# Rongjiehuang/FastDiff

Hardware: AMD Instinct MI355X
Metric: real-time factor (audio-sec/wall-sec), N=4 reverse steps, 80x864 mel (higher is better)
Workload: dtype f32 results; 2-piece fp16 operands (22 bit) on fp16 MFMA, fp32 accumulate; GEMM as Winograd F(2,3); exact-fp32 twin; 1 GPU; BASELINE configs[1]: LJSpeech shape, batch=8 x 80x864 mel per GPU, N=4, HIP kernels + hipGraph sampler; batch_per_gpu=8, frames=864, reverse_steps=4, graph=True, weights=random init seed 1234 (no checkpoint offline), world_size=1, gpus_visible=1, oversubscribed=False

## Files before the change

### fastdiff_amd/csrc/fd_api.cpp

```cpp
#include <math.h>
#include <stddef.h>
#include <stdio.h>
#include <stdlib.h>
#include <string.h>

#include <algorithm>

#include "fd_kernels.h"
#include "fd_host.h"

std::string g_create_error;

static inline int gx_rows_host(int T) { return std::max(fdk_fast::gx_rows(T), fdk_fast::gw_pairs(T) * (fdk_fast::GW_ROWB / fdk_fast::GX_ROWB)); }

bool fd_prof_stamps(const fdk::Launch &L, const char *name, hipEvent_t *e0, hipEvent_t *e1)
{
    fd_context *c = L.ctx;
    if (c->profile != 1 || L.capturing) return false;
    hipEvent_t ev[2];
    for (int i = 0; i < 2; ++i) {
        if (!c->event_pool.empty()) { ev[i] = c->event_pool.back(); c->event_pool.pop_back(); }
        else if (hipEventCreate(&ev[i]) != hipSuccess) return false;
    }
    ProfEntry pe;
// ... 300 lines not shown
    }
    for (int i = fuse_up ? 1 : 0; i < fd::LAYERS; ++i) {
        if (m.fast[ST_LVC]) {
            e = fast_lvc_layer(L, io, n, i, cur, skip, other, B, T);
            std::swap(cur, other);
        } else {
            e = naive_lvc_layer(L, n, i, cur, skip, other, B, T);
        }
        if (e != hipSuccess) return e;
    }
    if (m.keep_taps) {
        e = hipMemcpyAsync(ws.xtap[n], cur, sizeof(float) * (size_t)B * fd::C * T * fd::hop(n), hipMemcpyDeviceToDevice, L.stream);
        if (e != hipSuccess) return e;
    }
    *x_out = cur;
    return hipSuccess;
}

static hipError_t run_step(const Launch &L, const StepIO &io, int B, int T)
{
    Workspace &ws = L.ctx->ws;
    hipError_t e;
    const bool hoisted = L.mode->hoist_np > 1;
    if ((e = first_conv(L, io, B, T)) != hipSuccess) return e;
    for (int d = 0; d < fd::NBLK; ++d)
        if ((e = dblock(L, io, d, B, T)) != hipSuccess) return e;
    if (!hoisted) {
        if ((e = kp_front(L, io, B, T)) != hipSuccess) return e;
        if ((e = kp_gemm(L, B, T)) != hipSuccess) return e;
    }
    float *x = ws.a[3];
    for (int n = 0; n < fd::NBLK; ++n) {
        float *xo = nullptr;
        if ((e = lvc_block_run(L, io, n, x, B, T, &xo)) != hipSuccess) return e;
        x = xo;
    }
    if (L.mode->fast[ST_FINAL]) return fast_final(L, io, x, B, T);
    float *eps = io.sampler ? ((x == ws.xA) ? ws.xB : ws.xA) : io.eps_out;
    if ((e = naive_final_eps(L, x, eps, B, T)) != hipSuccess) return e;
    if (io.sampler) return naive_update(L, ws.x, eps, (int64_t)B * T * fd::HOPT);
    return hipSuccess;
}

}

extern "C" {


// ... 103 lines not shown
    if (e != hipSuccess) FD_FAIL(h, FD_ERR_HIP, "fd_forward: kernel launch failed: %s", hipGetErrorString(e));
    h->last_B = B; h->last_T = T;
    return fd_mark_tail(h, (hipStream_t)stream);
}

static int resolve_pending(fd_handle h, unsigned *mask);
int fd_settle(fd_handle h)
{
    if (!h->pending.active) return FD_OK;
    unsigned mask = 0;
    const int rc = resolve_pending(h, &mask);
    return rc < 0 ? rc : FD_OK;
}

static int enqueue_steps(fd_handle h, int B, int T, int count, const StepMode &mode, hipStream_t stream)
{
    Workspace &ws = h->ws;
    constexpr int CHUNK = 8;
    auto piece_mode = [&](int steps) {
        StepMode m = mode;
        if (m.hoist_chunk) m.hoist_np = steps;
        return m;
    };
    const bool defer_advance = mode.fuse_advance && mode.fast[ST_FIRST];
    auto enqueue_piece = [&](const fdk::Launch &L, int steps) -> hipError_t {
        const int np = L.mode->hoist_chunk ? L.mode->hoist_np : 1;
        hipError_t e = hipSuccess;
        if (np > 1) {
            StepIO iop = {ws.x, ws.mel_rep, nullptr, nullptr, np};
            e = fdk::kp_front(L, iop, B * np, T);
            if (e == hipSuccess) e = fdk::kp_gemm(L, B * np, T);
        }
        for (int k = 0; k < steps && e == hipSuccess; ++k) {
            StepIO io = {ws.x, ws.mel, nullptr, nullptr, 1};
            io.hoist_step = L.mode->hoist_np > 1 ? k : 0;
            io.advance = k > 0 && defer_advance;
            e = fdk::run_step(L, io, B, T);
            if (e == hipSuccess && !(k + 1 < steps && defer_advance)) e = fdk::advance_step(L);
        }
        return e;
    };
    if (!(h->use_graph && !h->profile)) {
        const int piece = mode.hoist_chunk ? CHUNK : count;
        for (int first = 0; first < count; first += piece) {
            const int steps = std::min(piece, count - first);
            const StepMode m = piece_mode(steps);
            const hipError_t e = enqueue_piece({h, stream, false, &m}, steps);
// ... 363 lines not shown
    static const char *stage_names[ST_COUNT] = {"embed", "first", "dblock", "kp_front", "kp_gemm", "convt", "lvc", "final"};
    auto parse_mode = [&](bool &dst) -> int {
        if (v == "fast") dst = true;
        else if (v == "naive") dst = false;
        else FD_FAIL(h, FD_ERR_INVALID, "fd_set_option: %s expects fast|naive, got '%s'", key, value);
        return FD_OK;
    };
    if (k == "kernels") {
        bool m = true;
        int rc = parse_mode(m);
        if (rc != FD_OK) return rc;
        for (int i = 0; i < ST_COUNT; ++i) h->mode.fast[i] = m;
        return FD_OK;
    }
    if (k.compare(0, 8, "kernels.") == 0) {
        for (int i = 0; i < ST_COUNT; ++i)
            if (k.substr(8) == stage_names[i]) return parse_mode(h->mode.fast[i]);
        FD_FAIL(h, FD_ERR_INVALID, "fd_set_option: unknown stage '%s'", key);
    }
    static const struct { const char *key, *a, *b; void (*set)(fd_context *, bool); } choices[] = {
        {"gemm", "f16x2", "fp32", [](fd_context *c, bool a) { c->mode.gemm_f16 = a; }},
        {"gemm_form", "winograd", "direct", [](fd_context *c, bool a) { c->mode.gemm_wino = a; }},
        {"gemm_tile", "16", "32", [](fd_context *c, bool a) { c->mode.gemm_tile16 = a; }},
        {"lvc", "f16x2", "fp32", [](fd_context *c, bool a) { c->mode.lvc_f16 = a; }},
        {"conv", "f16x2", "fp32", [](fd_context *c, bool a) { c->mode.conv_f16 = a; }},
        {"lvc_h8", "mfma", "valu", [](fd_context *c, bool a) { c->mode.lvc_h8_mfma = a; }},
        {"fallback", "graph", "host", [](fd_context *c, bool a) { c->host_fallback = !a; }},
        {"lvc_dx", "gather", "copy", [](fd_context *c, bool a) { c->lvc_dx_gather = a; }},
        {"mel", "pwg", "tacotron", [](fd_context *c, bool a) { c->mel_variant = a ? MEL_PWG : MEL_TACOTRON; }},
    };
    for (const auto &ch : choices) {
        if (k != ch.key) continue;
        if (v != ch.a && v != ch.b) FD_FAIL(h, FD_ERR_INVALID, "fd_set_option: %s expects %s|%s, got '%s'", key, ch.a, ch.b, value);
        ch.set(h, v == ch.a);
        return FD_OK;
    }
    const bool on = (v == "1" || v == "true" || v == "on");
    if (k == "fuse_final") { h->mode.fuse_final = on; return FD_OK; }
    if (k == "fuse_up") { h->mode.fuse_up = on; return FD_OK; }
    if (k == "fuse_advance") { h->mode.fuse_advance = on; return FD_OK; }
    if (k == "embed_cache") { h->embed_cache = on; return FD_OK; }
    if (k == "hoist") {
        if (v == "auto") h->hoist_mode = 1;
        else if (v == "on") h->hoist_mode = 2;
        else if (v == "off") h->hoist_mode = 0;
        else FD_FAIL(h, FD_ERR_INVALID, "fd_set_option: hoist expects auto|on|off, got '%s'", value);
// ... 20 lines not shown
```

### fastdiff_amd/csrc/fd_internal.h

```cpp
#pragma once
#include <hip/hip_runtime.h>
#include <hip/hip_ext.h>
#include <stdint.h>
#include <string.h>
#include <map>
#include <string>
#include <vector>

#include "../../include/fastdiff_hip.h"
#include "../../include/fastdiff_hip_ext.h"
#include "../../include/fastdiff_hip_train.h"

namespace fd {
constexpr int C = 32;
constexpr int COND = 80;
constexpr int HID = 64;
constexpr int NBLK = 3;
constexpr int LAYERS = 4;
constexpr int HOPT = 256;
constexpr int E_IN = 128, E_MID = 512, E_OUT = 512;
constexpr int KLAYER = 2 * C * C * 3;
constexpr int KW = KLAYER * LAYERS;
constexpr int KB = 2 * C * LAYERS;
constexpr int KREC = KW + KB;
// ... 58 lines not shown
    int n_steps;
    int ddim;
    int step_idx;
    int l4;
    const unsigned long long *uids;
    int l4_io;
    long long n4_io;
    const long long *offs4;
};

enum Stage { ST_EMBED = 0, ST_FIRST, ST_DBLOCK, ST_KP_FRONT, ST_KP_GEMM, ST_CONVT, ST_LVC, ST_FINAL, ST_COUNT };

struct StepMode {
    bool fast[ST_COUNT] = {true, true, true, true, true, true, true, true};
    bool gemm_f16 = true;
    bool gemm_wino = true;
    bool gemm_tile16 = true;
    bool lvc_f16 = true;
    bool conv_f16 = true;
    bool lvc_h8_mfma = true;
    bool fuse_final = true;
    bool fuse_up = true;
    bool fuse_advance = true;
    bool keep_taps = false;
    unsigned fp32_mask = 0;
    bool inline_fallback = true;
    bool ragged = false;
    int hoist_np = 1;
    bool hoist_chunk = false;

    bool operator==(const StepMode &o) const
    {
        for (int i = 0; i < ST_COUNT; ++i)
            if (fast[i] != o.fast[i]) return false;
        return gemm_f16 == o.gemm_f16 && gemm_wino == o.gemm_wino && gemm_tile16 == o.gemm_tile16 && lvc_f16 == o.lvc_f16 && conv_f16 == o.conv_f16 &&
               lvc_h8_mfma == o.lvc_h8_mfma && fuse_final == o.fuse_final && fuse_up == o.fuse_up && fuse_advance == o.fuse_advance &&
               keep_taps == o.keep_taps && fp32_mask == o.fp32_mask && inline_fallback == o.inline_fallback && ragged == o.ragged &&
               hoist_np == o.hoist_np && hoist_chunk == o.hoist_chunk;
    }
};

struct Workspace {
    int B = 0;
    int64_t frames = 0;
    int64_t rows = 0;
    float *noise = nullptr;
    float *embed_h2 = nullptr;
    float *a[4] = {};
    float *kp_h0 = nullptr, *kp_hA = nullptr, *kp_hB = nullptr;
    float *kpack = nullptr;
    float *h_f16 = nullptr;
    int *lens_dev = nullptr;
    unsigned long long *uid_dev = nullptr;
    long long *off_dev = nullptr;
    float *xsave = nullptr;
    int *range_flag = nullptr;
    float *xA = nullptr, *xB = nullptr;
    float *xtap[fd::NBLK] = {};
    int64_t pframes = 0, prows = 0, plens = 0;
    float *mel_rep = nullptr;
// ... 135 lines not shown
    Scratch step_scratch;
    std::vector<ProfEntry> prof_pending;
    std::vector<hipEvent_t> event_pool;
    std::map<std::string, std::pair<int64_t, double>> prof_acc;
};

enum Pipe { PIPE_F16_THEN_F32, PIPE_F16_ONLY, PIPE_F32_ONLY };
inline Pipe fd_pipe(const StepMode &m, bool f16_possible, int flag_word)
{
    if (!f16_possible || ((m.fp32_mask >> flag_word) & 1u)) return PIPE_F32_ONLY;
    return m.inline_fallback ? PIPE_F16_THEN_F32 : PIPE_F16_ONLY;
}
inline bool front_writes_h_image(const StepMode &m, const DevWeights &w)
{
    return m.fast[ST_KP_FRONT] && fd_pipe(m, m.conv_f16 && w.kpf_f16_ok, 19) != PIPE_F32_ONLY &&
           fd_pipe(m, m.gemm_f16 && w.gemm_f16_ok, 0) != PIPE_F32_ONLY && !(m.gemm_wino && w.gemm_w_ok);
}
inline bool last_lvc_fuses_final(const StepMode &m, const DevWeights &w)
{
    return m.fast[ST_LVC] && m.fast[ST_FINAL] && !m.keep_taps && m.fuse_final &&
           fd_pipe(m, m.lvc_f16 && w.lvc_f16_ok, 1 + 2 * fd::LAYERS + 3) != PIPE_F32_ONLY;
}

struct StepIO {
    const float *x_in;
    const float *mel;
    const float *steps;
    float *eps_out;
    int sampler;
    int hoist_step = 0;
    bool advance = false;
};

namespace fdk {
struct Launch {
    fd_context *ctx;
    hipStream_t stream;
    bool capturing;
    const StepMode *mode = nullptr;
};
hipError_t embed(const Launch &L, const StepIO &io, int B, int n_steps);
hipError_t first_conv(const Launch &L, const StepIO &io, int B, int T);
hipError_t dblock(const Launch &L, const StepIO &io, int d, int B, int T);
hipError_t kp_front(const Launch &L, const StepIO &io, int B, int T);
hipError_t kp_gemm(const Launch &L, int B, int T);
hipError_t advance_step(const Launch &L);
// ... 51 lines not shown
```

### fastdiff_amd/csrc/fd_kernels.h

```cpp
#pragma once
#include "fd_internal.h"

namespace fdk_fast {
constexpr int GX_CT = 4;
constexpr int GX_ROWB = 2 * 128;
constexpr int GW_PAIRS = 32;
constexpr int GW_ROWB = 1024;
__host__ __device__ inline int gx_rows(int T) { return ((T + GX_CT * 32 - 1) / (GX_CT * 32)) * (GX_CT * 32) + 2; }
__host__ __device__ inline int gw_pairs(int T) { return ((T + 2 * GW_PAIRS - 1) / (2 * GW_PAIRS)) * GW_PAIRS; }

__host__ __device__ inline int gw16_a_off(int lane, int q, int ks)
{
    const int r = lane & 15, g = lane >> 4;
    return r * GW_ROWB + (((8 * q + 4 * ks + g) ^ r) << 4);
}
__host__ __device__ inline int gw16_b_idx(int ptile, int q, int j, int ks, int ct, int lane)
{
    const int kh = 4 * ks + (lane >> 4);
    return ((ptile * 2 + q) * 16 + 4 * j + (kh >> 1)) * 64 + 32 * (kh & 1) + 16 * ct + (lane & 15);
}
__host__ __device__ inline int gw16_d_pair(int lane, int i) { return 4 * (lane >> 4) + i; }
__host__ __device__ inline int gw16_d_pos(int lane, int ct) { return 16 * ct + (lane & 15); }
__host__ __device__ inline unsigned gw16_st_lane_off(int lane) { return (unsigned)(16 * (lane >> 5)) * (unsigned)fd::KREC + (unsigned)(lane & 31); }
__host__ __device__ inline int gw16_st_row_off(int rt, int part, int i, int odd) { return (2 * (16 * rt + 4 * part + i) + odd) * fd::KREC; }
}

namespace fdk {
hipError_t naive_first_conv(const Launch &L, const StepIO &io, int B, int T);
hipError_t naive_dblock(const Launch &L, int d, int B, int T);
hipError_t naive_kp_front(const Launch &L, const StepIO &io, int B, int T);
hipError_t naive_kp_gemm(const Launch &L, int B, int T);
hipError_t naive_convt(const Launch &L, int n, const float *x_in, float *x_out, int B, int Lin);
hipError_t naive_lvc_layer(const Launch &L, int n, int layer, float *x, const float *skip, float *y, int B, int T);
hipError_t naive_final_eps(const Launch &L, const float *x32, float *eps, int B, int T);
hipError_t naive_update(const Launch &L, float *x, const float *eps, int64_t n);
hipError_t fast_first_conv(const Launch &L, const StepIO &io, int B, int T);
hipError_t fast_dblock(const Launch &L, int d, int B, int T, const float *audio);
hipError_t fast_kp_front(const Launch &L, const StepIO &io, int B, int T);
hipError_t fast_kp_gemm(const Launch &L, int B, int T);
hipError_t fast_convt(const Launch &L, int n, const float *x_in, float *x_out, int B, int Lin);
hipError_t fast_lvc_layer(const Launch &L, const StepIO &io, int n, int layer, const float *x_in, const float *skip, float *x_out, int B, int T,
                          bool up = false);
hipError_t fast_final(const Launch &L, const StepIO &io, const float *x32, int B, int T);
bool lvc_op_needs_scratch(int Cin, int Cout, int ks, int hop);
hipError_t lvc_op_forward(const Launch &L, const float *x, const float *K, const float *bias, float *out, int B, int Cin, int Cout, int ks,
                          int T, int hop, float *scratch, int64_t kbs = 0, bool frames = false, int64_t bbs = 0);
hipError_t lvc_op_backward(const Launch &L, const float *x, const float *K, const float *dout, float *dx, float *dK, float *dbias, int B,
                           int Cin, int Cout, int ks, int T, int hop, float *scratch, int64_t kbs = 0, int64_t dkbs = 0, bool frames = false,
                           int64_t dbbs = 0);
hipError_t gate_forward(const Launch &L, const float *x, const float *y, float *out, int B, int C, int64_t len);
hipError_t gate_backward(const Launch &L, const float *y, const float *dout, float *dy, int B, int C, int64_t len);
hipError_t fan_pick(const Launch &L, const float *x, float *out, int rows, int64_t len, int f);
hipError_t fan_sum(const Launch &L, const float *const g[4], const float *gp, float *dx, int rows, int64_t len, int f);
bool kconv_supported(int M, int T);
size_t kconv_scratch_floats(int B, int M, int T);
bool kconv_frames_supported(int M, int T);
bool kconv_act_supported(int M, int T);
hipError_t kconv_forward(const Launch &L, const float *h, const float *W, const float *bias, float *out, int B, int M, int T, bool frames = false,
                         float post = 1.0f);
hipError_t kconv_backward(const Launch &L, const float *h, const float *W, const float *dout, float *dh, float *dW, float *dbias, int B, int M,
// ... 105 lines not shown
```

### fastdiff_amd/csrc/fd_kernels_common.h

```cpp
#ifndef FD_KERNELS_COMMON_H
#define FD_KERNELS_COMMON_H
#include "fd_kernels.h"
#include "fd_device.h"

typedef float f32x16 __attribute__((ext_vector_type(16)));

namespace fdk_fast {

__device__ __forceinline__ f32x16 mfma32(float a, float b, f32x16 c)
{
    return __builtin_amdgcn_mfma_f32_32x32x2f32(a, b, c, 0, 0, 0);
}
__device__ __forceinline__ int drow(int r, int hi) { return (r & 3) + 8 * (r >> 2) + 4 * hi; }
__device__ __forceinline__ int opaque(int x)
{
    asm volatile("" : "+v"(x));
    return x;
}
__device__ __forceinline__ float lrelu(float v, float s)
{
    return __builtin_amdgcn_fmed3f(v, v * s, __builtin_inff());
}
__device__ __forceinline__ float f4c(const float4 &v, int r) { return r == 0 ? v.x : (r == 1 ? v.y : (r == 2 ? v.z : v.w)); }

__device__ __forceinline__ int frames_of(const int *lens, int b, int T) { return lens ? lens[b] : T; }

__device__ __forceinline__ bool skip_after_previous_overflow(int *flag)
{
    if (flag[32] == 0) return false;
    if (blockIdx.x == 0 && blockIdx.y == 0 && blockIdx.z == 0 && threadIdx.x == 0) atomicOr(flag, 1);
    return true;
}

constexpr float GX_SCALE = 2048.0f, GX_INV_SCALE = 1.0f / 2048.0f;
constexpr float GX_LIMIT = 32768.0f;
typedef _Float16 f16x8 __attribute__((ext_vector_type(8)));
__device__ __forceinline__ f32x16 mfma_f16(const float4 &a, const float4 &b, f32x16 c)
{
    union { float4 f; f16x8 h; } ua, ub;
    ua.f = a;
    ub.f = b;
    return __builtin_amdgcn_mfma_f32_32x32x16_f16(ua.h, ub.h, c, 0, 0, 0);
}

typedef _Float16 h2_t __attribute__((ext_vector_type(2)));
typedef float f2_t __attribute__((ext_vector_type(2)));

__device__ __forceinline__ void split2(float a, float b, unsigned &hi, unsigned &lo)
{
    const f2_t v = {a, b};
    const h2_t h = __builtin_convertvector(v, h2_t);
    const f2_t r = (v - __builtin_convertvector(h, f2_t)) * GX_SCALE;
    const h2_t l = __builtin_convertvector(r, h2_t);
    hi = __builtin_bit_cast(unsigned, h);
// ... 26 lines not shown


#ifndef FD_LVC_NT
#define FD_LVC_NT 66
#endif
typedef float lvc_f4 __attribute__((ext_vector_type(4)));
template <int BIT>
__device__ __forceinline__ float4 lvc_ld(const float4 *p)
{
    if constexpr ((FD_LVC_NT & BIT) != 0) {
        const lvc_f4 v = __builtin_nontemporal_load(reinterpret_cast<const lvc_f4 *>(p));
        return make_float4(v.x, v.y, v.z, v.w);
    } else return *p;
}
template <int BIT>
__device__ __forceinline__ void lvc_st(float *p, float v) { if constexpr ((FD_LVC_NT & BIT) != 0) __builtin_nontemporal_store(v, p); else *p = v; }
template <int BIT>
__device__ __forceinline__ void lvc_st(float4 *p, const float4 &v)
{
    if constexpr ((FD_LVC_NT & BIT) != 0) __builtin_nontemporal_store(lvc_f4{v.x, v.y, v.z, v.w}, reinterpret_cast<lvc_f4 *>(p));
    else *p = v;
}

#ifndef FD_LVC_XCD_RUN
#define FD_LVC_XCD_RUN 8
#endif
template <int R = FD_LVC_XCD_RUN>
__device__ __forceinline__ int lvc_tile_of_workgroup()
{
    constexpr int G = 8 * R;
    const int n = blockIdx.x;
    if constexpr (R <= 1) return n;
    const int g0 = (n / G) * G;
    return (g0 + G <= (int)gridDim.x) ? g0 + (n % 8) * R + (n / 8) % R : n;
}

}
#endif
```

### fastdiff_amd/csrc/fd_kernels_dblock.hip

```cpp
#include "fd_kernels_common.h"

namespace fdk_fast {

constexpr int DB_LD = 136;
constexpr int DB_STRIDE = 114;

template <int DIL, bool LRELU>
__device__ __forceinline__ void conv96_tile(f32x16 &acc, const float4 (&wa)[12], const float *in, int ld, int col, int hi)
{
    const int o[3] = {opaque(hi * ld + col - DIL), opaque(hi * ld + col), opaque(hi * ld + col + DIL)};
#pragma unroll
    for (int s = 0; s < 48; ++s) {
        const int tap = s >> 4, c2 = (2 * s) & 31;
        float v = in[o[tap] + c2 * ld];
        if (LRELU) v = lrelu(v, 0.2f);
        acc = mfma32(f4c(wa[s >> 2], s & 3), v, acc);
    }
}

template <int F>
__global__ void __launch_bounds__(256, 2) k_dblock(const float *__restrict__ xin, float *__restrict__ out,
                                                   const float *__restrict__ p0, const float *__restrict__ p1,
                                                   const float *__restrict__ p2, const float *__restrict__ pr,
                                                   const float *__restrict__ b0, const float *__restrict__ b1,
// ... 87 lines not shown
}
__device__ __forceinline__ void store_act_h2(char *img, const f32x16 &ah, const f32x16 &al, int c, int hi, bool inside, float &mx)
{
    const int row = 4 + c;
#pragma unroll
    for (int j = 0; j < 4; ++j) {
        float v[4];
#pragma unroll
        for (int i = 0; i < 4; ++i) {
            v[i] = inside ? lrelu(fmaf(al[4 * j + i], GX_INV_SCALE, ah[4 * j + i]), 0.2f) : 0.0f;
            mx = fmaxf(mx, fabsf(v[i]));
        }
        uint2 ph, pl;
        split2(v[0], v[1], ph.x, pl.x);
        split2(v[2], v[3], ph.y, pl.y);
        *reinterpret_cast<uint2 *>(img + h2_off(row, j) + 8 * hi) = ph;
        *reinterpret_cast<uint2 *>(img + h2_off(row, 4 + j) + 8 * hi) = pl;
    }
}

#ifndef FD_DBLOCK_OCC
#define FD_DBLOCK_OCC 3
#endif
template <int F, bool AUDIO>
__global__ void __launch_bounds__(256, FD_DBLOCK_OCC) k_dblock_h2(const float *__restrict__ xin, float *__restrict__ out,
                                                      const float4 *__restrict__ p0, const float4 *__restrict__ p1,
                                                      const float4 *__restrict__ p2, const float4 *__restrict__ pr,
                                                      const float *__restrict__ b0, const float *__restrict__ b1,
                                                      const float *__restrict__ b2, const float *__restrict__ br, int Lin, int Lo,
                                                      int *__restrict__ range_flag, const int *__restrict__ lens, int per_frame,
                                                      const float *__restrict__ audio, const float *__restrict__ fw,
                                                      const float *__restrict__ fb)
{
    __shared__ __attribute__((aligned(16))) char xl[DBH_ROWS * 128];
    __shared__ __attribute__((aligned(16))) char xr[DBH_ROWS * 128];
    __shared__ __attribute__((aligned(16))) char ha[DBH_ROWS * 128];
    const int b = blockIdx.y, tid = threadIdx.x, lane = tid & 63, wave = tid >> 6, l31 = lane & 31, hi = lane >> 5;
    const int pbase = blockIdx.x * DB_STRIDE - 7;
    const int Lob = lens ? lens[b] * per_frame : Lo;
    if (blockIdx.x * DB_STRIDE >= Lob || skip_after_previous_overflow(range_flag)) return;
    float mx = 0.0f;
    __shared__ float fwl[AUDIO ? 256 : 1];
    if constexpr (AUDIO) {
        fwl[tid] = tid < 224 ? fw[tid] : fb[tid - 224];
        __syncthreads();
    }
    {
        float v[2][8];
#pragma unroll
        for (int k = 0; k < 2; ++k) {
            const int u = k * 256 + tid, cg = u >> 7, cc = u & 127, p = pbase + cc;
            const bool ok = p >= 0 && p < Lob;
            if (AUDIO) {
                const int Lb = Lob * F, t = p * F;
                const float *xa = audio + (int64_t)b * Lin;
                float xv[7];
#pragma unroll
                for (int i = 0; i < 7; ++i) xv[i] = (ok && t - 3 + i >= 0 && t - 3 + i < Lb) ? xa[t - 3 + i] : 0.0f;
                const int o0 = __builtin_amdgcn_readfirstlane(cg) * 8;
#pragma unroll
                for (int c = 0; c < 8; ++c) {
                    float r = fwl[224 + o0 + c];
#pragma unroll
                    for (int i = 0; i < 7; ++i) r += fwl[(o0 + c) * 7 + i] * xv[i];
                    v[k][c] = ok ? r : 0.0f;
                }
            } else {
#pragma unroll
                for (int c = 0; c < 8; ++c) v[k][c] = ok ? xin[((int64_t)b * fd::C + cg * 8 + c) * Lin + (int64_t)p * F] : 0.0f;
            }
        }
        if (tid < 128) {
            const int g = tid >> 4, row = g < 4 ? g : 128 + g, part = tid & 15;
            *reinterpret_cast<uint2 *>(xl + row * 128 + part * 8) = make_uint2(0u, 0u);
            *reinterpret_cast<uint2 *>(xr + row * 128 + part * 8) = make_uint2(0u, 0u);
            *reinterpret_cast<uint2 *>(ha + row * 128 + part * 8) = make_uint2(0u, 0u);
        }
#pragma unroll
        for (int k = 0; k < 2; ++k) {
            const int u = k * 256 + tid, cg = u >> 7, cc = u & 127;
            float a[8];
#pragma unroll
            for (int c = 0; c < 8; ++c) { mx = fmaxf(mx, fabsf(v[k][c])); a[c] = lrelu(v[k][c], 0.2f); }
            float4 ph, pl;
            split8(v[k], ph, pl);
            *reinterpret_cast<float4 *>(xr + h2_off(4 + cc, cg)) = ph;
            *reinterpret_cast<float4 *>(xr + h2_off(4 + cc, 4 + cg)) = pl;
            split8(a, ph, pl);
            *reinterpret_cast<float4 *>(xl + h2_off(4 + cc, cg)) = ph;
            *reinterpret_cast<float4 *>(xl + h2_off(4 + cc, 4 + cg)) = pl;
        }
    }
    __syncthreads();
    const int c = wave * 32 + l31;
    const int p = pbase + c;
    const bool inside = (p >= 0 && p < Lob);
    float4 wa[2][6];
    f32x16 ah, al;
    auto load_w = [&](const float4 *pk) {
#pragma unroll
        for (int q = 0; q < 2; ++q)
#pragma unroll
            for (int kg = 0; kg < 6; ++kg) wa[q][kg] = pk[(q * 6 + kg) * 64 + lane];
    };
    load_w(p0);
#pragma unroll
    for (int r = 0; r < 16; ++r) { ah[r] = b0[drow(r, hi)]; al[r] = 0.0f; }
    conv96_h2<1>(ah, al, wa, xl, c, hi);
    store_act_h2(ha, ah, al, c, hi, inside, mx);
    __syncthreads();
    load_w(p1);
#pragma unroll
    for (int r = 0; r < 16; ++r) { ah[r] = b1[drow(r, hi)]; al[r] = 0.0f; }
    conv96_h2<2>(ah, al, wa, ha, c, hi);
    store_act_h2(xl, ah, al, c, hi, inside, mx);
    __syncthreads();
    load_w(p2);
#pragma unroll
    for (int r = 0; r < 16; ++r) { ah[r] = b2[drow(r, hi)] + br[drow(r, hi)]; al[r] = 0.0f; }
    conv96_h2<4>(ah, al, wa, xl, c, hi);
    {
        float4 wr[2][2];
#pragma unroll
        for (int q = 0; q < 2; ++q)
#pragma unroll
            for (int kg = 0; kg < 2; ++kg) wr[q][kg] = pr[(q * 2 + kg) * 64 + lane];
#pragma unroll
        for (int kg = 0; kg < 2; ++kg) {
            const float4 x1 = *reinterpret_cast<const float4 *>(xr + h2_off(4 + c, kg * 2 + hi));
            const float4 x2 = *reinterpret_cast<const float4 *>(xr + h2_off(4 + c, 4 + kg * 2 + hi));
            ah = mfma_f16(wr[0][kg], x1, ah);
            al = mfma_f16(wr[0][kg], x2, al);
            al = mfma_f16(wr[1][kg], x1, al);
        }
    }
    if (inside && c >= 7 && c < 7 + DB_STRIDE) {
#pragma unroll
        for (int r = 0; r < 16; ++r) out[((int64_t)b * fd::C + drow(r, hi)) * Lo + p] = fmaf(al[r], GX_INV_SCALE, ah[r]);
    }
    if (!(mx < GX_LIMIT)) atomicOr(range_flag, 1);
}

}

namespace fdk {
using namespace fdk_fast;

hipError_t fast_dblock(const Launch &L, int d, int B, int T, const float *audio)
{
    fd_context *c = L.ctx;
    const DevWeights &w = c->w;
    int Lin = T * fd::HOPT;
    for (int i = 0; i < d; ++i) Lin /= fd::down_factor(i);
    const int f = fd::down_factor(d), Lo = Lin / f;
    const dim3 grid((Lo + DB_STRIDE - 1) / DB_STRIDE, B);
    const int *run_if = nullptr;
    const char *n4 = "dblock_f4", *n8 = "dblock_f8";
    const int *lens = L.mode->ragged ? c->ws.lens_dev : nullptr;
    const Pipe pipe = fd_pipe(*L.mode, L.mode->conv_f16 && w.dblock_f16_ok, 13 + d);
    if (pipe != PIPE_F32_ONLY) {
        int *flag = c->ws.range_flag + 13 + d;
        const float4 *q0 = reinterpret_cast<const float4 *>(w.down_h2[d][0]), *q1 = reinterpret_cast<const float4 *>(w.down_h2[d][1]),
                     *q2 = reinterpret_cast<const float4 *>(w.down_h2[d][2]), *q3 = reinterpret_cast<const float4 *>(w.down_h2[d][3]);
// ... 3 lines not shown
                      w.down[d].conv[1].b, w.down[d].conv[2].b, w.down[d].res.b, Lin, Lo, flag, lens, Lo / T, audio,
                      (const float *)w.first.w, (const float *)w.first.b);
        else if (f == 4)
            FD_LAUNCH(L, n4, (k_dblock_h2<4, false>), grid, dim3(256), 0, c->ws.a[d], c->ws.a[d + 1], q0, q1, q2, q3, w.down[d].conv[0].b,
                      w.down[d].conv[1].b, w.down[d].conv[2].b, w.down[d].res.b, Lin, Lo, flag, lens, Lo / T, none, none, none);
        else
            FD_LAUNCH(L, n8, (k_dblock_h2<8, false>), grid, dim3(256), 0, c->ws.a[d], c->ws.a[d + 1], q0, q1, q2, q3, w.down[d].conv[0].b,
                      w.down[d].conv[1].b, w.down[d].conv[2].b, w.down[d].res.b, Lin, Lo, flag, lens, Lo / T, none, none, none);
        run_if = flag;
        n4 = n8 = "dblock_fp32_fallback";
        if (pipe == PIPE_F16_ONLY) return hipSuccess;
    }
    if (f == 4)
        FD_LAUNCH(L, n4, k_dblock<4>, grid, dim3(256), 0, c->ws.a[d], c->ws.a[d + 1], w.down_pack[d][0], w.down_pack[d][1],
                  w.down_pack[d][2], w.down_pack[d][3], w.down[d].conv[0].b, w.down[d].conv[1].b, w.down[d].conv[2].b,
                  w.down[d].res.b, Lin, Lo, run_if, lens, Lo / T);
    else
        FD_LAUNCH(L, n8, k_dblock<8>, grid, dim3(256), 0, c->ws.a[d], c->ws.a[d + 1], w.down_pack[d][0], w.down_pack[d][1],
                  w.down_pack[d][2], w.down_pack[d][3], w.down[d].conv[0].b, w.down[d].conv[1].b, w.down[d].conv[2].b,
                  w.down[d].res.b, Lin, Lo, run_if, lens, Lo / T);
    return hipSuccess;
}

}
```

### fastdiff_amd/csrc/fd_kernels_first_final.hip

```cpp
#include "fd_kernels_common.h"

namespace fdk_fast {

__global__ void __launch_bounds__(256) k_first_conv(const float *__restrict__ x, const float *__restrict__ w,
                                                    const float *__restrict__ bias, float *__restrict__ a0, int L,
                                                    const int *__restrict__ lens, StepParams *advance, int *__restrict__ range_flags)
{
    if (advance && blockIdx.x == 0 && blockIdx.y == 0) {
        if (threadIdx.x == 0) advance->step_idx += 1;
        if (threadIdx.x < 32) {
            const int f = range_flags[threadIdx.x];
            range_flags[32 + threadIdx.x] = f;
            range_flags[64 + threadIdx.x] |= f;
            range_flags[threadIdx.x] = 0;
        }
    }
    __shared__ float wl[fd::C * 8];
    {
        const int o = threadIdx.x >> 3, k = threadIdx.x & 7;
        wl[threadIdx.x] = k < 7 ? w[o * 7 + k] : bias[o];
        __syncthreads();
    }
    const int b = blockIdx.y;
    const int t0 = (blockIdx.x * 256 + threadIdx.x) * 4;
    const int Lb = lens ? lens[b] * fd::HOPT : L;
    if (t0 >= Lb) return;
    const float *xr = x + (int64_t)b * L;
    float xv[10];
#pragma unroll
    for (int i = 0; i < 10; ++i) {
        const int p = t0 - 3 + i;
        xv[i] = (p >= 0 && p < Lb) ? xr[p] : 0.0f;
    }
#pragma unroll 4
    for (int o = 0; o < fd::C; ++o) {
        float wv[7];
#pragma unroll
        for (int k = 0; k < 7; ++k) wv[k] = wl[o * 8 + k];
        const float bv = wl[o * 8 + 7];
        float4 r = make_float4(bv, bv, bv, bv);
#pragma unroll
        for (int k = 0; k < 7; ++k) {
            r.x += wv[k] * xv[k]; r.y += wv[k] * xv[k + 1]; r.z += wv[k] * xv[k + 2]; r.w += wv[k] * xv[k + 3];
        }
        lvc_st<64>(reinterpret_cast<float4 *>(a0 + ((int64_t)b * fd::C + o) * L + t0), r);
    }
}


__global__ void __launch_bounds__(256) k_final_acc(float *__restrict__ eps_acc, const float *__restrict__ bias, float *__restrict__ eps_out,
                                                   float *__restrict__ xstate, const StepParams *params, int sampler, int L,
                                                   const int *__restrict__ lens, const int *__restrict__ overflow)
{
    const int b = blockIdx.y;
    const int t0 = (blockIdx.x * 256 + threadIdx.x) * 4;
    const int Lb = lens ? lens[b] * fd::HOPT : L;
    if (t0 >= Lb) return;
    const int64_t i4 = ((int64_t)b * L + t0) >> 2;
    float4 acc = reinterpret_cast<const float4 *>(eps_acc)[i4];
    reinterpret_cast<float4 *>(eps_acc)[i4] = make_float4(0.f, 0.f, 0.f, 0.f);
    if (*overflow) return;
    const float bv = bias[0];
    acc = make_float4(acc.x + bv, acc.y + bv, acc.z + bv, acc.w + bv);
    if (!sampler) {
        reinterpret_cast<float4 *>(eps_out)[i4] = acc;
    } else {
        const float4 xv = reinterpret_cast<const float4 *>(xstate)[i4];
        reinterpret_cast<float4 *>(xstate)[i4] = fdk::sampler_update4(xv, acc, params, b, (int64_t)(t0 >> 2));
    }
// ... 80 lines not shown
```

Baseline: 10140 x real-time.

## Co-schedule first conv and first downsample block in one interleaved launch

Adds a combined kernel whose 1-D grid interleaves blocks of the first dblock (which recomputes the first conv from audio inline) with blocks of the first conv that write a0 for later consumers. This removes one launch and the dependency between the two, so both can run concurrently on the GPU. Deferred sampler-advance fusion is turned off while this path is active, which may add a separate advance launch. The body code is factored into shared device functions so the old kernels keep working.

```diff
diff --git a/fastdiff_amd/csrc/fd_api.cpp b/fastdiff_amd/csrc/fd_api.cpp
--- a/fastdiff_amd/csrc/fd_api.cpp
+++ b/fastdiff_amd/csrc/fd_api.cpp
@@ -346,8 +346,11 @@
     Workspace &ws = L.ctx->ws;
     hipError_t e;
     const bool hoisted = L.mode->hoist_np > 1;
-    if ((e = first_conv(L, io, B, T)) != hipSuccess) return e;
-    for (int d = 0; d < fd::NBLK; ++d)
+    const bool pair_a = io.sampler && pair_a_active(*L.mode, L.ctx->w);
+    if (pair_a) {
+        if ((e = fast_pair_dblock_first(L, io, B, T)) != hipSuccess) return e;
+    } else if ((e = first_conv(L, io, B, T)) != hipSuccess) return e;
+    for (int d = pair_a ? 1 : 0; d < fd::NBLK; ++d)
         if ((e = dblock(L, io, d, B, T)) != hipSuccess) return e;
     if (!hoisted) {
         if ((e = kp_front(L, io, B, T)) != hipSuccess) return e;
@@ -497,7 +500,7 @@
         if (m.hoist_chunk) m.hoist_np = steps;
         return m;
     };
-    const bool defer_advance = mode.fuse_advance && mode.fast[ST_FIRST];
+    const bool defer_advance = mode.fuse_advance && mode.fast[ST_FIRST] && !pair_a_active(mode, h->w);
     auto enqueue_piece = [&](const fdk::Launch &L, int steps) -> hipError_t {
         const int np = L.mode->hoist_chunk ? L.mode->hoist_np : 1;
         hipError_t e = hipSuccess;
@@ -907,6 +910,7 @@
         {"gemm", "f16x2", "fp32", [](fd_context *c, bool a) { c->mode.gemm_f16 = a; }},
         {"gemm_form", "winograd", "direct", [](fd_context *c, bool a) { c->mode.gemm_wino = a; }},
         {"gemm_tile", "16", "32", [](fd_context *c, bool a) { c->mode.gemm_tile16 = a; }},
+        {"pair_head", "1", "0", [](fd_context *c, bool a) { c->mode.pair_head = a; }},
         {"lvc", "f16x2", "fp32", [](fd_context *c, bool a) { c->mode.lvc_f16 = a; }},
         {"conv", "f16x2", "fp32", [](fd_context *c, bool a) { c->mode.conv_f16 = a; }},
         {"lvc_h8", "mfma", "valu", [](fd_context *c, bool a) { c->mode.lvc_h8_mfma = a; }},
diff --git a/fastdiff_amd/csrc/fd_internal.h b/fastdiff_amd/csrc/fd_internal.h
--- a/fastdiff_amd/csrc/fd_internal.h
+++ b/fastdiff_amd/csrc/fd_internal.h
@@ -104,6 +104,7 @@
     bool fuse_final = true;
     bool fuse_up = true;
     bool fuse_advance = true;
+    bool pair_head = true;
     bool keep_taps = false;
     unsigned fp32_mask = 0;
     bool inline_fallback = true;
@@ -117,7 +118,8 @@
             if (fast[i] != o.fast[i]) return false;
         return gemm_f16 == o.gemm_f16 && gemm_wino == o.gemm_wino && gemm_tile16 == o.gemm_tile16 && lvc_f16 == o.lvc_f16 && conv_f16 == o.conv_f16 &&
                lvc_h8_mfma == o.lvc_h8_mfma && fuse_final == o.fuse_final && fuse_up == o.fuse_up && fuse_advance == o.fuse_advance &&
-               keep_taps == o.keep_taps && fp32_mask == o.fp32_mask && inline_fallback == o.inline_fallback && ragged == o.ragged &&
+               pair_head == o.pair_head && keep_taps == o.keep_taps && fp32_mask == o.fp32_mask &&
+               inline_fallback == o.inline_fallback && ragged == o.ragged &&
                hoist_np == o.hoist_np && hoist_chunk == o.hoist_chunk;
     }
 };
@@ -299,6 +301,11 @@
            fd_pipe(m, m.lvc_f16 && w.lvc_f16_ok, 1 + 2 * fd::LAYERS + 3) != PIPE_F32_ONLY;
 }
 
+inline bool pair_a_active(const StepMode &m, const DevWeights &w)
+{
+    return m.pair_head && m.fast[ST_FIRST] && m.fast[ST_DBLOCK] && fd_pipe(m, m.conv_f16 && w.dblock_f16_ok, 13) == PIPE_F16_ONLY;
+}
+
 struct StepIO {
     const float *x_in;
     const float *mel;
diff --git a/fastdiff_amd/csrc/fd_kernels.h b/fastdiff_amd/csrc/fd_kernels.h
--- a/fastdiff_amd/csrc/fd_kernels.h
+++ b/fastdiff_amd/csrc/fd_kernels.h
@@ -23,6 +23,35 @@
 __host__ __device__ inline int gw16_d_pos(int lane, int ct) { return 16 * ct + (lane & 15); }
 __host__ __device__ inline unsigned gw16_st_lane_off(int lane) { return (unsigned)(16 * (lane >> 5)) * (unsigned)fd::KREC + (unsigned)(lane & 31); }
 __host__ __device__ inline int gw16_st_row_off(int rt, int part, int i, int odd) { return (2 * (16 * rt + 4 * part + i) + odd) * fd::KREC; }
+
+struct PairGrid {
+    int g0, rows0, g1, rows1;
+    __host__ __device__ int n0() const { return g0 * rows0; }
+    __host__ __device__ int n1() const { return g1 * rows1; }
+    __host__ __device__ int total() const { return n0() + n1(); }
+};
+struct PairBlock { int role, bx, by; };
+__host__ __device__ inline PairBlock pair_block(const PairGrid &g, int role, int i) { return {role, i % (role ? g.g1 : g.g0), i / (role ? g.g1 : g.g0)}; }
+constexpr int PAIR_DB_STRIDE = 114, PAIR_FC_SAMPLES = 1024;
+constexpr int PAIR_A_P0 = 9, PAIR_A_P1 = 4;
+__host__ __device__ inline PairGrid pair_a_grid(int B, int T)
+{
+    return {(64 * T + PAIR_DB_STRIDE - 1) / PAIR_DB_STRIDE, B, (256 * T + PAIR_FC_SAMPLES - 1) / PAIR_FC_SAMPLES, B};
+}
+__host__ __device__ inline PairBlock pair_a_block(const PairGrid &g, int n)
+{
+    constexpr int P = PAIR_A_P0 + PAIR_A_P1;
+    const int n0 = g.n0(), n1 = g.n1();
+    const int q0 = n0 / PAIR_A_P0, q1 = n1 / PAIR_A_P1, periods = q0 < q1 ? q0 : q1;
+    if (n < periods * P) {
+        const int k = n / P, j = n - k * P;
+        if (j % 3 == 2) return pair_block(g, 1, k * PAIR_A_P1 + j / 3);
+        return pair_block(g, 0, k * PAIR_A_P0 + j - (j + 1) / 3);
+    }
+    const int m = n - periods * P, left0 = n0 - periods * PAIR_A_P0;
+    if (m < left0) return pair_block(g, 0, periods * PAIR_A_P0 + m);
+    return pair_block(g, 1, periods * PAIR_A_P1 + (m - left0));
+}
 }
 
 namespace fdk {
@@ -36,6 +65,7 @@
 hipError_t naive_update(const Launch &L, float *x, const float *eps, int64_t n);
 hipError_t fast_first_conv(const Launch &L, const StepIO &io, int B, int T);
 hipError_t fast_dblock(const Launch &L, int d, int B, int T, const float *audio);
+hipError_t fast_pair_dblock_first(const Launch &L, const StepIO &io, int B, int T);
 hipError_t fast_kp_front(const Launch &L, const StepIO &io, int B, int T);
 hipError_t fast_kp_gemm(const Launch &L, int B, int T);
 hipError_t fast_convt(const Launch &L, int n, const float *x_in, float *x_out, int B, int Lin);
diff --git a/fastdiff_amd/csrc/fd_kernels_common.h b/fastdiff_amd/csrc/fd_kernels_common.h
--- a/fastdiff_amd/csrc/fd_kernels_common.h
+++ b/fastdiff_amd/csrc/fd_kernels_common.h
@@ -25,11 +25,15 @@
 
 __device__ __forceinline__ int frames_of(const int *lens, int b, int T) { return lens ? lens[b] : T; }
 
+__device__ __forceinline__ bool skip_after_previous_overflow(int *flag, bool first_block)
+{
+    if (flag[32] == 0) return false;
+    if (first_block && threadIdx.x == 0) atomicOr(flag, 1);
+    return true;
+}
 __device__ __forceinline__ bool skip_after_previous_overflow(int *flag)
 {
-    if (flag[32] == 0) return false;
-    if (blockIdx.x == 0 && blockIdx.y == 0 && blockIdx.z == 0 && threadIdx.x == 0) atomicOr(flag, 1);
-    return true;
+    return skip_after_previous_overflow(flag, blockIdx.x == 0 && blockIdx.y == 0 && blockIdx.z == 0);
 }
 
 constexpr float GX_SCALE = 2048.0f, GX_INV_SCALE = 1.0f / 2048.0f;
@@ -102,6 +106,41 @@
     else *p = v;
 }
 
+__device__ __forceinline__ void first_conv_body(int bx, int by, float *__restrict__ wl , const float *__restrict__ x,
+                                                const float *__restrict__ w, const float *__restrict__ bias, float *__restrict__ a0, int L,
+                                                const int *__restrict__ lens)
+{
+    {
+        const int o = threadIdx.x >> 3, k = threadIdx.x & 7;
+        wl[threadIdx.x] = k < 7 ? w[o * 7 + k] : bias[o];
+        __syncthreads();
+    }
+    const int b = by;
+    const int t0 = (bx * 256 + threadIdx.x) * 4;
+    const int Lb = lens ? lens[b] * fd::HOPT : L;
+    if (t0 >= Lb) return;
+    const float *xr = x + (int64_t)b * L;
+    float xv[10];
+#pragma unroll
+    for (int i = 0; i < 10; ++i) {
+        const int p = t0 - 3 + i;
+        xv[i] = (p >= 0 && p < Lb) ? xr[p] : 0.0f;
+    }
+#pragma unroll 4
+    for (int o = 0; o < fd::C; ++o) {
+        float wv[7];
+#pragma unroll
+        for (int k = 0; k < 7; ++k) wv[k] = wl[o * 8 + k];
+        const float bv = wl[o * 8 + 7];
+        float4 r = make_float4(bv, bv, bv, bv);
+#pragma unroll
+        for (int k = 0; k < 7; ++k) {
+            r.x += wv[k] * xv[k]; r.y += wv[k] * xv[k + 1]; r.z += wv[k] * xv[k + 2]; r.w += wv[k] * xv[k + 3];
+        }
+        lvc_st<64>(reinterpret_cast<float4 *>(a0 + ((int64_t)b * fd::C + o) * L + t0), r);
+    }
+}
+
 #ifndef FD_LVC_XCD_RUN
 #define FD_LVC_XCD_RUN 8
 #endif
diff --git a/fastdiff_amd/csrc/fd_kernels_dblock.hip b/fastdiff_amd/csrc/fd_kernels_dblock.hip
--- a/fastdiff_amd/csrc/fd_kernels_dblock.hip
+++ b/fastdiff_amd/csrc/fd_kernels_dblock.hip
@@ -133,6 +133,126 @@
 #ifndef FD_DBLOCK_OCC
 #define FD_DBLOCK_OCC 3
 #endif
+constexpr int DBH_LDS = 3 * DBH_ROWS * 128 + 1024;
+template <int F, bool AUDIO>
+__device__ __forceinline__ void dblock_h2_body(int bx, int by, char *__restrict__ lds, const float *__restrict__ xin, float *__restrict__ out,
+                                               const float4 *__restrict__ p0, const float4 *__restrict__ p1,
+                                               const float4 *__restrict__ p2, const float4 *__restrict__ pr,
+                                               const float *__restrict__ b0, const float *__restrict__ b1,
+                                               const float *__restrict__ b2, const float *__restrict__ br, int Lin, int Lo,
+                                               int *__restrict__ range_flag, const int *__restrict__ lens, int per_frame,
+                                               const float *__restrict__ audio, const float *__restrict__ fw,
+                                               const float *__restrict__ fb)
+{
+    char *xl = lds;
+    char *xr = lds + DBH_ROWS * 128;
+    char *ha = lds + 2 * DBH_ROWS * 128;
+    const int b = by, tid = threadIdx.x, lane = tid & 63, wave = tid >> 6, l31 = lane & 31, hi = lane >> 5;
+    const int pbase = bx * DB_STRIDE - 7;
+    const int Lob = lens ? lens[b] * per_frame : Lo;
+    if (bx * DB_STRIDE >= Lob || skip_after_previous_overflow(range_flag, bx == 0 && by == 0)) return;
+    float mx = 0.0f;
+    float *fwl = reinterpret_cast<float *>(lds + 3 * DBH_ROWS * 128);
+    if constexpr (AUDIO) {
+        fwl[tid] = tid < 224 ? fw[tid] : fb[tid - 224];
+        __syncthreads();
+    }
+    {
+        float v[2][8];
+#pragma unroll
+        for (int k = 0; k < 2; ++k) {
+            const int u = k * 256 + tid, cg = u >> 7, cc = u & 127, p = pbase + cc;
+            const bool ok = p >= 0 && p < Lob;
+            if (AUDIO) {
+                const int Lb = Lob * F, t = p * F;
+                const float *xa = audio + (int64_t)b * Lin;
+                float xv[7];
+#pragma unroll
+                for (int i = 0; i < 7; ++i) xv[i] = (ok && t - 3 + i >= 0 && t - 3 + i < Lb) ? xa[t - 3 + i] : 0.0f;
+                const int o0 = __builtin_amdgcn_readfirstlane(cg) * 8;
+#pragma unroll
+                for (int c = 0; c < 8; ++c) {
+                    float r = fwl[224 + o0 + c];
+#pragma unroll
+                    for (int i = 0; i < 7; ++i) r += fwl[(o0 + c) * 7 + i] * xv[i];
+                    v[k][c] = ok ? r : 0.0f;
+                }
+            } else {
+#pragma unroll
+                for (int c = 0; c < 8; ++c) v[k][c] = ok ? xin[((int64_t)b * fd::C + cg * 8 + c) * Lin + (int64_t)p * F] : 0.0f;
+            }
+        }
+        if (tid < 128) {
+            const int g = tid >> 4, row = g < 4 ? g : 128 + g, part = tid & 15;
+            *reinterpret_cast<uint2 *>(xl + row * 128 + part * 8) = make_uint2(0u, 0u);
+            *reinterpret_cast<uint2 *>(xr + row * 128 + part * 8) = make_uint2(0u, 0u);
+            *reinterpret_cast<uint2 *>(ha + row * 128 + part * 8) = make_uint2(0u, 0u);
+        }
+#pragma unroll
+        for (int k = 0; k < 2; ++k) {
+            const int u = k * 256 + tid, cg = u >> 7, cc = u & 127;
+            float a[8];
+#pragma unroll
+            for (int c = 0; c < 8; ++c) { mx = fmaxf(mx, fabsf(v[k][c])); a[c] = lrelu(v[k][c], 0.2f); }
+            float4 ph, pl;
+            split8(v[k], ph, pl);
+            *reinterpret_cast<float4 *>(xr + h2_off(4 + cc, cg)) = ph;
+            *reinterpret_cast<float4 *>(xr + h2_off(4 + cc, 4 + cg)) = pl;
+            split8(a, ph, pl);
+            *reinterpret_cast<float4 *>(xl + h2_off(4 + cc, cg)) = ph;
+            *reinterpret_cast<float4 *>(xl + h2_off(4 + cc, 4 + cg)) = pl;
+        }
+    }
+    __syncthreads();
+    const int c = wave * 32 + l31;
+    const int p = pbase + c;
+    const bool inside = (p >= 0 && p < Lob);
+    float4 wa[2][6];
+    f32x16 ah, al;
+    auto load_w = [&](const float4 *pk) {
+#pragma unroll
+        for (int q = 0; q < 2; ++q)
+#pragma unroll
+            for (int kg = 0; kg < 6; ++kg) wa[q][kg] = pk[(q * 6 + kg) * 64 + lane];
+    };
+    load_w(p0);
+#pragma unroll
+    for (int r = 0; r < 16; ++r) { ah[r] = b0[drow(r, hi)]; al[r] = 0.0f; }
+    conv96_h2<1>(ah, al, wa, xl, c, hi);
+    store_act_h2(ha, ah, al, c, hi, inside, mx);
+    __syncthreads();
+    load_w(p1);
+#pragma unroll
+    for (int r = 0; r < 16; ++r) { ah[r] = b1[drow(r, hi)]; al[r] = 0.0f; }
+    conv96_h2<2>(ah, al, wa, ha, c, hi);
+    store_act_h2(xl, ah, al, c, hi, inside, mx);
+    __syncthreads();
+    load_w(p2);
+#pragma unroll
+    for (int r = 0; r < 16; ++r) { ah[r] = b2[drow(r, hi)] + br[drow(r, hi)]; al[r] = 0.0f; }
+    conv96_h2<4>(ah, al, wa, xl, c, hi);
+    {
+        float4 wr[2][2];
+#pragma unroll
+        for (int q = 0; q < 2; ++q)
+#pragma unroll
+            for (int kg = 0; kg < 2; ++kg) wr[q][kg] = pr[(q * 2 + kg) * 64 + lane];
+#pragma unroll
+        for (int kg = 0; kg < 2; ++kg) {
+            const float4 x1 = *reinterpret_cast<const float4 *>(xr + h2_off(4 + c, kg * 2 + hi));
+            const float4 x2 = *reinterpret_cast<const float4 *>(xr + h2_off(4 + c, 4 + kg * 2 + hi));
+            ah = mfma_f16(wr[0][kg], x1, ah);
+            al = mfma_f16(wr[0][kg], x2, al);
+            al = mfma_f16(wr[1][kg], x1, al);
+        }
+    }
+    if (inside && c >= 7 && c < 7 + DB_STRIDE) {
+#pragma unroll
+        for (int r = 0; r < 16; ++r) out[((int64_t)b * fd::C + drow(r, hi)) * Lo + p] = fmaf(al[r], GX_INV_SCALE, ah[r]);
+    }
+    if (!(mx < GX_LIMIT)) atomicOr(range_flag, 1);
+}
+
 template <int F, bool AUDIO>
 __global__ void __launch_bounds__(256, FD_DBLOCK_OCC) k_dblock_h2(const float *__restrict__ xin, float *__restrict__ out,
                                                       const float4 *__restrict__ p0, const float4 *__restrict__ p1,
@@ -143,113 +263,26 @@
                                                       const float *__restrict__ audio, const float *__restrict__ fw,
                                                       const float *__restrict__ fb)
 {
-    __shared__ __attribute__((aligned(16))) char xl[DBH_ROWS * 128];
-    __shared__ __attribute__((aligned(16))) char xr[DBH_ROWS * 128];
-    __shared__ __attribute__((aligned(16))) char ha[DBH_ROWS * 128];
-    const int b = blockIdx.y, tid = threadIdx.x, lane = tid & 63, wave = tid >> 6, l31 = lane & 31, hi = lane >> 5;
-    const int pbase = blockIdx.x * DB_STRIDE - 7;
-    const int Lob = lens ? lens[b] * per_frame : Lo;
-    if (blockIdx.x * DB_STRIDE >= Lob || skip_after_previous_overflow(range_flag)) return;
-    float mx = 0.0f;
-    __shared__ float fwl[AUDIO ? 256 : 1];
-    if constexpr (AUDIO) {
-        fwl[tid] = tid < 224 ? fw[tid] : fb[tid - 224];
-        __syncthreads();
-    }
-    {
-        float v[2][8];
-#pragma unroll
-        for (int k = 0; k < 2; ++k) {
-            const int u = k * 256 + tid, cg = u >> 7, cc = u & 127, p = pbase + cc;
-            const bool ok = p >= 0 && p < Lob;
-            if (AUDIO) {
-                const int Lb = Lob * F, t = p * F;
-                const float *xa = audio + (int64_t)b * Lin;
-                float xv[7];
-#pragma unroll
-                for (int i = 0; i < 7; ++i) xv[i] = (ok && t - 3 + i >= 0 && t - 3 + i < Lb) ? xa[t - 3 + i] : 0.0f;
-                const int o0 = __builtin_amdgcn_readfirstlane(cg) * 8;
-#pragma unroll
-                for (int c = 0; c < 8; ++c) {
-                    float r = fwl[224 + o0 + c];
-#pragma unroll
-                    for (int i = 0; i < 7; ++i) r += fwl[(o0 + c) * 7 + i] * xv[i];
-                    v[k][c] = ok ? r : 0.0f;
-                }
-            } else {
-#pragma unroll
-                for (int c = 0; c < 8; ++c) v[k][c] = ok ? xin[((int64_t)b * fd::C + cg * 8 + c) * Lin + (int64_t)p * F] : 0.0f;
-            }
-        }
-        if (tid < 128) {
-            const int g = tid >> 4, row = g < 4 ? g : 128 + g, part = tid & 15;
-            *reinterpret_cast<uint2 *>(xl + row * 128 + part * 8) = make_uint2(0u, 0u);
-            *reinterpret_cast<uint2 *>(xr + row * 128 + part * 8) = make_uint2(0u, 0u);
-            *reinterpret_cast<uint2 *>(ha + row * 128 + part * 8) = make_uint2(0u, 0u);
-        }
-#pragma unroll
-        for (int k = 0; k < 2; ++k) {
-            const int u = k * 256 + tid, cg = u >> 7, cc = u & 127;
-            float a[8];
-#pragma unroll
-            for (int c = 0; c < 8; ++c) { mx = fmaxf(mx, fabsf(v[k][c])); a[c] = lrelu(v[k][c], 0.2f); }
-            float4 ph, pl;
-            split8(v[k], ph, pl);
-            *reinterpret_cast<float4 *>(xr + h2_off(4 + cc, cg)) = ph;
-            *reinterpret_cast<float4 *>(xr + h2_off(4 + cc, 4 + cg)) = pl;
-            split8(a, ph, pl);
-            *reinterpret_cast<float4 *>(xl + h2_off(4 + cc, cg)) = ph;
-            *reinterpret_cast<float4 *>(xl + h2_off(4 + cc, 4 + cg)) = pl;
-        }
-    }
-    __syncthreads();
-    const int c = wave * 32 + l31;
-    const int p = pbase + c;
-    const bool inside = (p >= 0 && p < Lob);
-    float4 wa[2][6];
-    f32x16 ah, al;
-    auto load_w = [&](const float4 *pk) {
-#pragma unroll
-        for (int q = 0; q < 2; ++q)
-#pragma unroll
-            for (int kg = 0; kg < 6; ++kg) wa[q][kg] = pk[(q * 6 + kg) * 64 + lane];
-    };
-    load_w(p0);
-#pragma unroll
-    for (int r = 0; r < 16; ++r) { ah[r] = b0[drow(r, hi)]; al[r] = 0.0f; }
-    conv96_h2<1>(ah, al, wa, xl, c, hi);
-    store_act_h2(ha, ah, al, c, hi, inside, mx);
-    __syncthreads();
-    load_w(p1);
-#pragma unroll
-    for (int r = 0; r < 16; ++r) { ah[r] = b1[drow(r, hi)]; al[r] = 0.0f; }
-    conv96_h2<2>(ah, al, wa, ha, c, hi);
-    store_act_h2(xl, ah, al, c, hi, inside, mx);
-    __syncthreads();
-    load_w(p2);
-#pragma unroll
-    for (int r = 0; r < 16; ++r) { ah[r] = b2[drow(r, hi)] + br[drow(r, hi)]; al[r] = 0.0f; }
-    conv96_h2<4>(ah, al, wa, xl, c, hi);
-    {
-        float4 wr[2][2];
-#pragma unroll
-        for (int q = 0; q < 2; ++q)
-#pragma unroll
-            for (int kg = 0; kg < 2; ++kg) wr[q][kg] = pr[(q * 2 + kg) * 64 + lane];
-#pragma unroll
-        for (int kg = 0; kg < 2; ++kg) {
-            const float4 x1 = *reinterpret_cast<const float4 *>(xr + h2_off(4 + c, kg * 2 + hi));
-            const float4 x2 = *reinterpret_cast<const float4 *>(xr + h2_off(4 + c, 4 + kg * 2 + hi));
-            ah = mfma_f16(wr[0][kg], x1, ah);
-            al = mfma_f16(wr[0][kg], x2, al);
-            al = mfma_f16(wr[1][kg], x1, al);
-        }
-    }
-    if (inside && c >= 7 && c < 7 + DB_STRIDE) {
-#pragma unroll
-        for (int r = 0; r < 16; ++r) out[((int64_t)b * fd::C + drow(r, hi)) * Lo + p] = fmaf(al[r], GX_INV_SCALE, ah[r]);
-    }
-    if (!(mx < GX_LIMIT)) atomicOr(range_flag, 1);
+    __shared__ __attribute__((aligned(16))) char lds[AUDIO ? DBH_LDS : 3 * DBH_ROWS * 128];
+    dblock_h2_body<F, AUDIO>(blockIdx.x, blockIdx.y, lds, xin, out, p0, p1, p2, pr, b0, b1, b2, br, Lin, Lo, range_flag, lens, per_frame, audio,
+                             fw, fb);
+}
+
+__global__ void __launch_bounds__(256, FD_DBLOCK_OCC) k_pair_dblock_first(
+    float *__restrict__ a0, float *__restrict__ out, const float4 *__restrict__ p0, const float4 *__restrict__ p1,
+    const float4 *__restrict__ p2, const float4 *__restrict__ pr, const float *__restrict__ b0, const float *__restrict__ b1,
+    const float *__restrict__ b2, const float *__restrict__ br, int Lin, int Lo, int *__restrict__ range_flag,
+    const int *__restrict__ lens, int per_frame, const float *__restrict__ audio, const float *__restrict__ fw,
+    const float *__restrict__ fb, int B, int T)
+{
+    static_assert(PAIR_DB_STRIDE == DB_STRIDE && PAIR_FC_SAMPLES == 4 * 256, "fd_kernels.h: pair_a_grid");
+    __shared__ __attribute__((aligned(16))) char lds[DBH_LDS];
+    const PairBlock r = pair_a_block(pair_a_grid(B, T), (int)blockIdx.x);
+    if (r.role == 0)
+        dblock_h2_body<4, true>(r.bx, r.by, lds, a0, out, p0, p1, p2, pr, b0, b1, b2, br, Lin, Lo, range_flag, lens, per_frame,
+                                audio, fw, fb);
+    else
+        first_conv_body(r.bx, r.by, reinterpret_cast<float *>(lds), audio, fw, fb, a0, Lin, lens);
 }
 
 }
@@ -299,4 +332,18 @@
     return hipSuccess;
 }
 
-}
+hipError_t fast_pair_dblock_first(const Launch &L, const StepIO &io, int B, int T)
+{
+    fd_context *c = L.ctx;
+    const DevWeights &w = c->w;
+    const int Lin = T * fd::HOPT, Lo = Lin / 4;
+    const int *lens = L.mode->ragged ? c->ws.lens_dev : nullptr;
+    FD_LAUNCH(L, "k_pair_dblock_first", k_pair_dblock_first, dim3(pair_a_grid(B, T).total()), dim3(256), 0, c->ws.a[0], c->ws.a[1],
+              reinterpret_cast<const float4 *>(w.down_h2[0][0]), reinterpret_cast<const float4 *>(w.down_h2[0][1]),
+              reinterpret_cast<const float4 *>(w.down_h2[0][2]), reinterpret_cast<const float4 *>(w.down_h2[0][3]), w.down[0].conv[0].b,
+              w.down[0].conv[1].b, w.down[0].conv[2].b, w.down[0].res.b, Lin, Lo, c->ws.range_flag + 13, lens, Lo / T, io.x_in,
+              (const float *)w.first.w, (const float *)w.first.b, B, T);
+    return hipSuccess;
+}
+
+}
diff --git a/fastdiff_amd/csrc/fd_kernels_first_final.hip b/fastdiff_amd/csrc/fd_kernels_first_final.hip
--- a/fastdiff_amd/csrc/fd_kernels_first_final.hip
+++ b/fastdiff_amd/csrc/fd_kernels_first_final.hip
@@ -16,35 +16,7 @@
         }
     }
     __shared__ float wl[fd::C * 8];
-    {
-        const int o = threadIdx.x >> 3, k = threadIdx.x & 7;
-        wl[threadIdx.x] = k < 7 ? w[o * 7 + k] : bias[o];
-        __syncthreads();
-    }
-    const int b = blockIdx.y;
-    const int t0 = (blockIdx.x * 256 + threadIdx.x) * 4;
-    const int Lb = lens ? lens[b] * fd::HOPT : L;
-    if (t0 >= Lb) return;
-    const float *xr = x + (int64_t)b * L;
-    float xv[10];
-#pragma unroll
-    for (int i = 0; i < 10; ++i) {
-        const int p = t0 - 3 + i;
-        xv[i] = (p >= 0 && p < Lb) ? xr[p] : 0.0f;
-    }
-#pragma unroll 4
-    for (int o = 0; o < fd::C; ++o) {
-        float wv[7];
-#pragma unroll
-        for (int k = 0; k < 7; ++k) wv[k] = wl[o * 8 + k];
-        const float bv = wl[o * 8 + 7];
-        float4 r = make_float4(bv, bv, bv, bv);
-#pragma unroll
-        for (int k = 0; k < 7; ++k) {
-            r.x += wv[k] * xv[k]; r.y += wv[k] * xv[k + 1]; r.z += wv[k] * xv[k + 2]; r.w += wv[k] * xv[k + 3];
-        }
-        lvc_st<64>(reinterpret_cast<float4 *>(a0 + ((int64_t)b * fd::C + o) * L + t0), r);
-    }
+    first_conv_body(blockIdx.x, blockIdx.y, wl, x, w, bias, a0, L, lens);
 }
 
 
```

Measured after the change: 10210 x real-time, median of 6. About the same (+0.7%).
